# ChristianFeldmann/libHM

Measured on AMD Instinct MI355X. Metric: decoded Mpixels/s (luma), 2160p Main10 reconstruction + loop filters, higher is better.
Workload: dtype int16 samples / int32 accumulate; 1 GPU; 3840x2160 Main10 lowdelay_P pictures, pre-parsed CTU metadata: prep+MC+dequant/IT/recon+deblock+SAO, batch of 16 independent pictures per step, inputs resident in HBM; sub_benchmark=full, streams=2, parallelism=frame-parallel, 1 process per GPU, no data-path collective

## Files before the change

include/hmgpu.h:

```cpp
#ifndef HMGPU_H
#define HMGPU_H

#include <stddef.h>
#include <stdint.h>

#ifdef __cplusplus
extern "C" {
#endif

#define HMGPU_VERSION 1

typedef enum hmgpu_status {
  HMGPU_OK = 0,
  HMGPU_EINVAL = 1,
  HMGPU_EDEVICE = 2,
  HMGPU_EUNSUPPORTED = 3,
  HMGPU_ENOMEM = 4
} hmgpu_status;

#define HMGPU_MAX_REF 16
#define HMGPU_MAX_SLICES 600
#define HMGPU_NO_PIC (-1)

enum { HMGPU_B_SLICE = 0, HMGPU_P_SLICE = 1, HMGPU_I_SLICE = 2 };
// ... 101 lines not shown
void* hmgpu_host_alloc(size_t bytes);
void  hmgpu_host_free(void* p);

int32_t hmgpu_num_ctus(const hmgpu_seq_params* seq);
int32_t hmgpu_parts_per_ctu(const hmgpu_seq_params* seq);

hmgpu_status hmgpu_picture_acquire(hmgpu_ctx* ctx, hmgpu_pic* out);
hmgpu_status hmgpu_picture_release(hmgpu_ctx* ctx, hmgpu_pic pic);
hmgpu_status hmgpu_picture_upload(hmgpu_ctx* ctx, hmgpu_pic pic, const int16_t* const planes[3], const int32_t strides[3]);
hmgpu_status hmgpu_picture_download(hmgpu_ctx* ctx, hmgpu_pic pic, int16_t* const planes[3], const int32_t strides[3]);

hmgpu_status hmgpu_picture_download_begin(hmgpu_ctx* ctx, hmgpu_pic pic, int16_t* const planes[3], const int32_t strides[3], uint64_t* ticket);
hmgpu_status hmgpu_download_wait(hmgpu_ctx* ctx, uint64_t ticket);

hmgpu_status hmgpu_picture_download_packed(hmgpu_ctx* ctx, hmgpu_pic pic, void* const planes[3], const int32_t stride_bytes[3],
                                           int32_t bytes_per_sample, int32_t crop_left, int32_t crop_right, int32_t crop_top, int32_t crop_bottom);
hmgpu_status hmgpu_picture_hash(hmgpu_ctx* ctx, hmgpu_pic pic, int32_t method, uint8_t digest[3][16], int32_t* digest_len);
hmgpu_status hmgpu_picture_hash_begin(hmgpu_ctx* ctx, hmgpu_pic pic, int32_t method , uint64_t* ticket);
hmgpu_status hmgpu_hash_wait(hmgpu_ctx* ctx, uint64_t ticket, int32_t block, uint8_t digest[3][16], int32_t* digest_len, int32_t* ready);

typedef enum { HMGPU_REGION_FINISHED = 0, HMGPU_REGION_RECEIVE = 1 } hmgpu_region;
hmgpu_status hmgpu_picture_transfer(hmgpu_ctx* src, hmgpu_pic src_pic, hmgpu_ctx* dst, hmgpu_pic dst_pic);
uint64_t     hmgpu_transfer_bytes(const hmgpu_ctx* ctx);
hmgpu_status hmgpu_picture_device_region(hmgpu_ctx* ctx, hmgpu_pic pic, int32_t which, void** base, int64_t* bytes);
hmgpu_status hmgpu_picture_commit_received(hmgpu_ctx* ctx, hmgpu_pic pic);
void* hmgpu_stream(hmgpu_ctx* ctx);

enum { HMGPU_EXPORT_PLANAR = 0, HMGPU_EXPORT_SEMIPLANAR = 1, HMGPU_EXPORT_RGB = 2 };
typedef struct hmgpu_export_desc {
  int32_t layout;
  int32_t bit_depth[2];
  int32_t bytes_per_sample;
  int32_t msb_aligned;
  int32_t crop[4];
  int32_t matrix, full_range;
  int32_t reserved[6];
} hmgpu_export_desc;
typedef struct hmgpu_export_plan {
  int32_t planes;
  int32_t width[3], height[3];
  int32_t row_bytes[3];
  int32_t coef[16];
} hmgpu_export_plan;
hmgpu_status hmgpu_export_plan_for(const hmgpu_seq_params* seq, const hmgpu_export_desc* desc, hmgpu_export_plan* out);
hmgpu_status hmgpu_picture_export(hmgpu_ctx* ctx, hmgpu_pic pic, const hmgpu_export_desc* desc, void* const dst[3],
                                  const int64_t pitch_bytes[3], int32_t on_stream, void* stream);
// ... 194 lines not shown
```

libhm_amd/__init__.py:

```python
import ctypes as C
import os

import numpy as np

from . import abi

_HERE = os.path.dirname(os.path.abspath(__file__))
LIB_PATH = os.path.join(_HERE, "libhmgpu.so")
_lib = None


class HmgpuError(RuntimeError):
    def __init__(self, status, what, device_error=0):
        self.status = status
        self.device_error = device_error
        names = {1: "HMGPU_EINVAL", 2: "HMGPU_EDEVICE", 3: "HMGPU_EUNSUPPORTED", 4: "HMGPU_ENOMEM"}
        super().__init__("%s failed: %s%s" % (what, names.get(status, status),
                                              " (hipError %d)" % device_error if status == 2 else ""))


def _share_torch_hip_runtime():
    import importlib.util
    import sys
    if "torch" in sys.modules:
# ... 21 lines not shown
        L = C.CDLL(LIB_PATH)
        L.hmgpu_create.argtypes = [C.POINTER(abi.SeqParams), C.c_int, C.POINTER(C.c_void_p)]
        L.hmgpu_destroy.argtypes = [C.c_void_p]
        L.hmgpu_destroy.restype = None
        L.hmgpu_last_device_error.argtypes = [C.c_void_p]
        L.hmgpu_debug_stall_intra.argtypes = [C.c_void_p, C.c_int32, C.c_int32]
        L.hmgpu_sync.argtypes = [C.c_void_p]
        L.hmgpu_status_string.restype = C.c_char_p
        L.hmgpu_kernel_name.restype = C.c_char_p
        L.hmgpu_num_ctus.argtypes = [C.POINTER(abi.SeqParams)]
        L.hmgpu_parts_per_ctu.argtypes = [C.POINTER(abi.SeqParams)]
        L.hmgpu_picture_acquire.argtypes = [C.c_void_p, C.POINTER(C.c_int32)]
        L.hmgpu_picture_release.argtypes = [C.c_void_p, C.c_int32]
        L.hmgpu_picture_upload.argtypes = [C.c_void_p, C.c_int32, C.POINTER(C.c_void_p), C.POINTER(C.c_int32)]
        L.hmgpu_picture_download.argtypes = [C.c_void_p, C.c_int32, C.POINTER(C.c_void_p), C.POINTER(C.c_int32)]
        L.hmgpu_set_streams.argtypes = [C.c_void_p, C.c_int32]
        L.hmgpu_picture_download_packed.argtypes = [C.c_void_p, C.c_int32, C.POINTER(C.c_void_p), C.POINTER(C.c_int32)] + [C.c_int32] * 5
        L.hmgpu_picture_hash.argtypes = [C.c_void_p, C.c_int32, C.c_int32, C.c_void_p, C.POINTER(C.c_int32)]
        L.hmgpu_picture_device_region.argtypes = [C.c_void_p, C.c_int32, C.c_int32, C.POINTER(C.c_void_p), C.POINTER(C.c_int64)]
        L.hmgpu_picture_commit_received.argtypes = [C.c_void_p, C.c_int32]
        L.hmgpu_picture_transfer.argtypes = [C.c_void_p, C.c_int32, C.c_void_p, C.c_int32]
        L.hmgpu_transfer_bytes.argtypes = [C.c_void_p]
        L.hmgpu_transfer_bytes.restype = C.c_uint64
        L.hmgpu_export_plan_for.argtypes = [C.POINTER(abi.SeqParams), C.POINTER(abi.ExportDesc), C.POINTER(abi.ExportPlan)]
        L.hmgpu_picture_export.argtypes = [C.c_void_p, C.c_int32, C.POINTER(abi.ExportDesc), C.POINTER(C.c_void_p), C.POINTER(C.c_int64),
                                           C.c_int32, C.c_void_p]
        L.hmgpu_export_scaled_plan_for.argtypes = [C.POINTER(abi.SeqParams), C.POINTER(abi.ExportDesc), C.POINTER(abi.ExportScale),
                                                   C.POINTER(abi.ExportPlan)]
        L.hmgpu_export_scale_taps.argtypes = [C.POINTER(abi.SeqParams), C.POINTER(abi.ExportDesc), C.POINTER(abi.ExportScale), C.c_int32,
                                              C.c_int32, C.c_int32, C.POINTER(C.c_int32), C.POINTER(C.c_int32), C.POINTER(C.c_int16)]
        L.hmgpu_picture_export_scaled.argtypes = [C.c_void_p, C.c_int32, C.POINTER(abi.ExportDesc), C.POINTER(abi.ExportScale),
                                                  C.POINTER(C.c_void_p), C.POINTER(C.c_int64), C.c_int32, C.c_void_p]
        L.hmgpu_export_tensor_plan_for.argtypes = [C.POINTER(abi.SeqParams), C.POINTER(abi.ExportDesc), C.POINTER(abi.ExportScale),
                                                   C.POINTER(abi.ExportTensor), C.POINTER(abi.ExportPlan)]
        L.hmgpu_pictures_export.argtypes = [C.c_void_p, C.c_int32, C.POINTER(C.c_int32), C.POINTER(abi.ExportDesc), C.POINTER(abi.ExportScale),
                                            C.POINTER(abi.ExportTensor), C.POINTER(C.c_void_p), C.POINTER(C.c_int64), C.POINTER(C.c_int64),
                                            C.c_int32, C.c_void_p]
        L.hmgpu_export_destination_check.argtypes = [C.c_void_p, C.c_int32, C.POINTER(abi.ExportDesc), C.POINTER(abi.ExportScale),
                                                     C.POINTER(abi.ExportTensor), C.POINTER(C.c_void_p), C.POINTER(C.c_int64),
                                                     C.POINTER(C.c_int64)]
        L.hmgpu_export_windows_plan_for.argtypes = [C.POINTER(abi.SeqParams), C.POINTER(abi.ExportDesc), C.POINTER(abi.ExportScale),
                                                    C.POINTER(abi.ExportTensor), C.c_int32, C.POINTER(abi.ExportWindow),
                                                    C.POINTER(abi.ExportPlan)]
        L.hmgpu_pictures_export_windows.argtypes = [C.c_void_p, C.c_int32, C.POINTER(C.c_int32), C.POINTER(abi.ExportDesc),
                                                    C.POINTER(abi.ExportScale), C.POINTER(abi.ExportTensor), C.POINTER(abi.ExportWindow),
                                                    C.POINTER(C.c_void_p), C.POINTER(C.c_int64), C.POINTER(C.c_int64), C.c_int32, C.c_void_p]
# ... 412 lines not shown

    def picture_hash(self, pic, method):
        dig = (C.c_uint8 * 48)()
        n = C.c_int32()
        self._chk(lib().hmgpu_picture_hash(self._h, pic, method, dig, C.byref(n)), "hmgpu_picture_hash")
        return np.array([dig[16 * k + i] for k in range(3) for i in range(n.value)], dtype=np.uint8)

    def device_region(self, pic, receive=False):
        base, nbytes = C.c_void_p(), C.c_int64()
        self._chk(lib().hmgpu_picture_device_region(self._h, pic, 1 if receive else 0, C.byref(base), C.byref(nbytes)),
                  "hmgpu_picture_device_region")
        return int(base.value), int(nbytes.value)

    def commit_received(self, pic):
        self._chk(lib().hmgpu_picture_commit_received(self._h, pic), "hmgpu_picture_commit_received")

    def transfer_to(self, pic, other, other_pic):
        self._chk(lib().hmgpu_picture_transfer(self._h, pic, other._h, other_pic), "hmgpu_picture_transfer")

    @property
    def transfer_bytes(self):
        return int(lib().hmgpu_transfer_bytes(self._h))

    def stream_handle(self):
        return int(lib().hmgpu_stream(self._h) or 0)

    def decompress_slice(self, pic, slice_idx, slice_params, meta, coeffs, first_ctu=0, num_ctus=None):
        n = self.num_ctus - first_ctu if num_ctus is None else num_ctus
        st = lib().hmgpu_decompress_slice(self._h, pic, slice_idx, C.byref(slice_params), C.byref(meta.struct),
                                          C.byref(coeffs.struct), first_ctu, n)
        self._chk(st, "hmgpu_decompress_slice")

    def filter_picture(self, pic, pic_params, sao_raw=None, stages=7):
        arr = abi.sao_array_from_raw(sao_raw) if sao_raw is not None else None
        st = lib().hmgpu_filter_picture_stages(self._h, pic, C.byref(pic_params), arr, stages)
        self._chk(st, "hmgpu_filter_picture_stages")

    @staticmethod
    def picture_jobs(jobs):
        arr = (abi.PictureJob * len(jobs))()
        arr._keep = [jobs]
        for i, (pic, slices, meta, coeffs) in enumerate(jobs):
            sl = (C.POINTER(abi.SliceParams) * len(slices))(*[C.pointer(s) for s in slices])
            arr._keep.append(sl)
            arr[i].pic, arr[i].num_slices, arr[i].slices = pic, len(slices), sl
            arr[i].meta = C.pointer(meta.struct)
# ... 98 lines not shown
```

libhm_amd/csrc/hmgpu_api.hip:

```cpp
#include "hmgpu_host.h"

#include <algorithm>
#include <cstdio>
#include <cstring>
#include <cstdlib>
#include <new>
#include <vector>

namespace hmgpu_host __attribute__((visibility("hidden"))) {

hipError_t h2d_small(hmgpu_ctx* c, void* dst, const void* src, size_t bytes, hipStream_t hs) {
  const size_t need = (bytes + 63) & ~(size_t)63;
  if (!c->bounce || need > hmgpu_ctx::kBounceSeg) return hipMemcpyAsync(dst, src, bytes, hipMemcpyHostToDevice, hs);
  if (c->bounce_off + need > hmgpu_ctx::kBounceSeg) {
    hipStream_t streams[3] = {c->stream, c->copy_stream, c->copy_stream2};
    for (int k = 0; k < 3; k++) (void)hipEventRecord(c->bounce_ev[c->bounce_seg][k], streams[k]);
    c->bounce_used[c->bounce_seg] = true;
    c->bounce_seg = (c->bounce_seg + 1) % hmgpu_ctx::kBounceSegs;
    c->bounce_off = 0;
    if (c->bounce_used[c->bounce_seg]) for (int k = 0; k < 3; k++) (void)hipEventSynchronize(c->bounce_ev[c->bounce_seg][k]);
  }
  char* at = c->bounce + (size_t)c->bounce_seg * hmgpu_ctx::kBounceSeg + c->bounce_off;
  memcpy(at, src, bytes);
  c->bounce_off += need;
// ... 200 lines not shown
  if (p.derived) hipFree(p.derived);
  p.planes = p.meta = p.coef = p.derived = nullptr; p.pcm = nullptr;
}

hmgpu_status ensure_refs_extended(hmgpu_ctx* c, const Batch& b, size_t call_idx) {
  for (int i = 0; i < b.n; i++) {
    const Picture& p = c->pics[b.pic[i]];
    if (call_idx >= p.calls.size()) continue;
    const SliceDev& sd = p.slices[p.calls[call_idx].slice_idx];
    for (int l = 0; l < 2; l++)
      for (int r = 0; r < HMGPU_MAX_REF; r++)
        if (sd.ref_pic[l][r] >= 0) { hmgpu_status st = ensure_extended(c, sd.ref_pic[l][r]); if (st != HMGPU_OK) return st; }
  }
  return HMGPU_OK;
}

}

namespace hmgpu_host __attribute__((visibility("hidden"))) {

hmgpu_status run_recon(hmgpu_ctx* c, const Batch& b, bool any_intra, bool any_wp, bool any_cells, bool any_bi, bool any_islice) {
  int max_ctus = 0;
  for (int i = 0; i < b.n; i++) max_ctus = std::max(max_ctus, b.num_ctus[i]);
  { ProfScope ps(c, K_PREP); launch_prep(c->d_pics, b, max_ctus, c->parts, any_intra, any_bi, any_cells || c->fmt != 1, c->fmt, c->stream); }
  if (c->fmt != 1) {
    for (int i = 0; i < b.n; i++) {
      const PicDev& d = c->pics[b.pic[i]].dev;
      HIP_TRY(c, hipMemsetAsync(d.resid[1], 0, (size_t)((char*)d.resid[2] - (char*)d.resid[1]) + c->coef_elems[2] * sizeof(int16_t), c->stream));
    }
  }
  McArgs ma;
  memset(&ma, 0, sizeof(ma));
  ma.n = b.n; ma.width = c->seq.width; ma.height = c->seq.height; ma.log2ctu = c->seq.log2_ctu_size; ma.ctus_w = c->ctus_w;
  ma.tw = c->grid_w / 2; ma.npics = c->seq.max_pictures;
  ma.slab = c->plane_slab; ma.pic_stride = 2 * c->plane_bytes; ma.slab_bytes = ma.pic_stride * c->pics.size(); ma.sao_off = (uint32_t)c->plane_bytes;
  for (size_t i = 0; i < c->pics.size(); i++)
    if (c->pics[i].sao_applied) (i < 32 ? ma.sao_mask_lo : ma.sao_mask_hi) |= 1u << (i & 31);
  for (int i = 0; i < b.n; i++) {
    const PicDev& d = c->pics[b.pic[i]].dev;
    ma.first_ctu[i] = b.first_ctu[i]; ma.num_ctus[i] = b.num_ctus[i];
    ma.tmv[i] = d.tmv; ma.slices[i] = d.slices;
  }
  const PicDev& d0 = c->pics[b.pic[0]].dev;
  const char* const base0 = (const char*)c->pics[b.pic[0]].planes;
  uint32_t bps = (uint32_t)std::max(4, std::min(b.n >= 4 ? 12 : 24, max_ctus / 8 + 1));
  {
    ItxArgs ia;
// ... 142 lines not shown
}
const char* hmgpu_kernel_name(int32_t k) { return (k >= 0 && k < HMGPU_NUM_KERNELS) ? kKernelNames[k] : ""; }

int32_t hmgpu_num_ctus(const hmgpu_seq_params* seq) {
  const int c = 1 << seq->log2_ctu_size;
  return ((seq->width + c - 1) / c) * ((seq->height + c - 1) / c);
}
int32_t hmgpu_parts_per_ctu(const hmgpu_seq_params* seq) { return 1 << (2 * seq->log2_ctu_size - 4); }

hmgpu_status hmgpu_create(const hmgpu_seq_params* seq, int device_ordinal, hmgpu_ctx** out) {
  if (!seq || !out) return HMGPU_EINVAL;
  *out = nullptr;
  if (seq->width <= 0 || seq->height <= 0 || (seq->width & 7) || (seq->height & 7)) return HMGPU_EINVAL;
  if (seq->log2_ctu_size < 4 || seq->log2_ctu_size > 6) return HMGPU_EINVAL;
  if (seq->max_pictures < 1 || seq->max_pictures > kMaxPics) return HMGPU_EINVAL;
  if (seq->chroma_format < 0 || seq->chroma_format > 3) return HMGPU_EINVAL;
  if (seq->range_ext_flags & ~(HMGPU_REXT_ROTATION | HMGPU_REXT_IMPLICIT_RDPCM | HMGPU_REXT_EXPLICIT_RDPCM | HMGPU_REXT_INTRA_SMOOTHING_DISABLED)) return HMGPU_EUNSUPPORTED;
  if (seq->bit_depth_luma < 8 || seq->bit_depth_luma > 12 || seq->bit_depth_chroma < 8 || seq->bit_depth_chroma > 12) return HMGPU_EUNSUPPORTED;
  hmgpu_ctx* c = new (std::nothrow) hmgpu_ctx();
  if (!c) return HMGPU_ENOMEM;
  c->seq = *seq;
  c->device = device_ordinal;
  c->host_timing = getenv("HMGPU_HOST_TIMING") != nullptr;
  hipError_t e = hipSetDevice(device_ordinal);
  if (e == hipSuccess) e = hipStreamCreateWithFlags(&c->stream, hipStreamNonBlocking);
  if (e == hipSuccess) e = hipStreamCreateWithFlags(&c->stream2, hipStreamNonBlocking);
  if (e == hipSuccess) e = hipStreamCreateWithFlags(&c->copy_stream, hipStreamNonBlocking);
  if (e == hipSuccess) e = hipStreamCreateWithFlags(&c->copy_stream2, hipStreamNonBlocking);
  if (e == hipSuccess) e = hipEventCreateWithFlags(&c->copy_join, hipEventDisableTiming);
  if (e == hipSuccess) e = hipHostMalloc((void**)&c->bounce, hmgpu_ctx::kBounceSegs * hmgpu_ctx::kBounceSeg, hipHostMallocDefault);
  for (int g = 0; g < hmgpu_ctx::kBounceSegs && e == hipSuccess; g++)
    for (int k = 0; k < 3 && e == hipSuccess; k++) e = hipEventCreateWithFlags(&c->bounce_ev[g][k], hipEventDisableTiming);
  for (int k = 0; k < 8 && e == hipSuccess; k++) e = hipEventCreateWithFlags(&c->copy_ev[k], hipEventDisableTiming);
  for (int k = 0; k < 8 && e == hipSuccess; k++) e = hipEventCreateWithFlags(&c->use_ev[k], hipEventDisableTiming);
  for (int k = 0; k < 32 && e == hipSuccess; k++) e = hipEventCreateWithFlags(&c->dl_ev[k], hipEventDisableTiming | hipEventBlockingSync);
  if (e == hipSuccess) { e = hipHostMalloc((void**)&c->dl_fault, 32 * sizeof(uint32_t), hipHostMallocDefault); if (e == hipSuccess) memset(c->dl_fault, 0, 32 * sizeof(uint32_t)); }
  for (int k = 0; k < 2 && e == hipSuccess; k++) e = hipEventCreateWithFlags(&c->lane_ev[k], hipEventDisableTiming);
  if (e != hipSuccess) { delete c; return HMGPU_EDEVICE; }
  c->ctu = 1 << seq->log2_ctu_size; c->pw = c->ctu / 4; c->parts = c->pw * c->pw;
  c->ctus_w = (seq->width + c->ctu - 1) / c->ctu; c->ctus_h = (seq->height + c->ctu - 1) / c->ctu;
  c->num_ctus = c->ctus_w * c->ctus_h;
  c->grid_w = c->ctus_w * c->pw; c->grid_h = c->ctus_h * c->pw;
  c->fmt = seq->chroma_format == 0 ? 1 : seq->chroma_format;
  c->csx = c->fmt == 3 ? 0 : 1; c->csy = c->fmt == 1 ? 1 : 0;
  c->mx[0] = 128; c->mx[1] = c->mx[2] = 128 >> c->csx;
  c->my[0] = 80; c->my[1] = c->my[2] = 80 >> c->csy;
// ... 264 lines not shown
    int can = 0;
    if (hipDeviceCanAccessPeer(&can, dst->device, src->device) == hipSuccess && can) {
      hipSetDevice(dst->device);
      const hipError_t e = hipDeviceEnablePeerAccess(src->device, 0);
      if (e != hipSuccess && e != hipErrorPeerAccessAlreadyEnabled) return HMGPU_EDEVICE;
      (void)hipGetLastError();
    }
  }
  hipSetDevice(src->device);
  if (!src->xfer_ev[0]) for (int k = 0; k < 2; k++) HIP_TRY(src, hipEventCreateWithFlags(&src->xfer_ev[k], hipEventDisableTiming));
  HIP_TRY(src, hipEventRecord(src->xfer_ev[0], src->stream));
  hipSetDevice(dst->device);
  HIP_TRY(dst, hipStreamWaitEvent(dst->stream, src->xfer_ev[0], 0));
  HIP_TRY(dst, hipMemcpyPeerAsync(to, dst->device, from, src->device, (size_t)n_from, dst->stream));
  HIP_TRY(dst, hipEventRecord(src->xfer_ev[1], dst->stream));
  hipSetDevice(src->device);
  HIP_TRY(src, hipStreamWaitEvent(src->stream, src->xfer_ev[1], 0));
  src->xfer_bytes += (uint64_t)n_from;
  touch(src, src_pic); commit_use(src);
  touch(dst, dst_pic); commit_use(dst);
  return hmgpu_picture_commit_received(dst, dst_pic);
}
uint64_t hmgpu_transfer_bytes(const hmgpu_ctx* c) { return c ? c->xfer_bytes : 0; }

void* hmgpu_stream(hmgpu_ctx* c) { return c ? (void*)c->stream : nullptr; }

hmgpu_status hmgpu_replay_batch(hmgpu_ctx* c, const hmgpu_pic* pics, int32_t n, int32_t stages, int32_t iters) {
  if (!c || !pics || n < 1 || n > kMaxBatch || iters < 0) return HMGPU_EINVAL;
  size_t ncalls = 0;
  for (int i = 0; i < n; i++) {
    if (!valid_pic(c, pics[i])) return HMGPU_EINVAL;
    if (i == 0) ncalls = c->pics[pics[i]].calls.size();
    else if (c->pics[pics[i]].calls.size() != ncalls) return HMGPU_EINVAL;
  }
  if ((stages & 8) && ncalls == 0) return HMGPU_EINVAL;
  hipSetDevice(c->device);
  const int lanes = (c->replay_streams == 2 && n >= 2 && !c->profiling) ? 2 : 1;
  hipStream_t const main_stream = c->stream;
  if (lanes == 2) {
    HIP_TRY(c, hipEventRecord(c->lane_ev[0], main_stream));
    HIP_TRY(c, hipStreamWaitEvent(c->stream2, c->lane_ev[0], 0));
  }
  hmgpu_status result = HMGPU_OK;
  for (int it = 0; it < iters && result == HMGPU_OK; it++) {
    for (int lane = 0; lane < lanes && result == HMGPU_OK; lane++) {
      const int lo = lanes == 2 ? (lane == 0 ? 0 : n / 2) : 0, hi = lanes == 2 ? (lane == 0 ? n / 2 : n) : n;
// ... 144 lines not shown
```

libhm_amd/csrc/hmgpu_dev.h:

```cpp
#pragma once
#include <hip/hip_runtime.h>
#include <stdint.h>
#include "../../include/hmgpu.h"

namespace hmgpu {

constexpr int kMaxBatch = 16;
constexpr int kMaxPics = 64;
constexpr int kTuShards = 8;
constexpr int kCStep = 2;

struct __attribute__((aligned(16))) BlkInfo {
  int16_t mv[2][2];
  int8_t  ref[2];
  int8_t  qp;
  uint8_t flags;
  uint8_t edge;
  uint8_t log2cu;
  uint16_t slice;
};
static_assert(sizeof(BlkInfo) == 16, "BlkInfo must be 16 bytes");

enum : uint8_t {
  BF_VALID = 1,
// ... 173 lines not shown
  if (n <= 8 && (8 % n) == 0) {
    const int m = 8 / n;
    const int per = (nb + m - 1) / m;
    const int x = bid & 7, t = bid >> 3;
    slot = x % n;
    const int r = x / n;
    lb = r * per + t;
    return t < per && lb < nb;
  }
  slot = bid % n; lb = bid / n;
  return lb < nb;
}
__host__ inline int xcd_grid(int n, int nb) {
  if (n <= 8 && (8 % n) == 0) { const int m = 8 / n; return 8 * ((nb + m - 1) / m); }
  return n * nb;
}

struct UnpackArgs {
  int32_t n;
  int32_t pic[kMaxBatch];
  const char* blob[kMaxBatch];
};
void launch_unpack_input(const PicDev* pics, const UnpackArgs& ua, int num_ctus, hipStream_t s);
void launch_prep(const PicDev* pics, const Batch& b, int max_ctus, int parts, bool intra, bool bi, bool write_blk, int fmt, hipStream_t s);
void launch_mc_luma(McArgs& a, int max_ctus, bool wp, bool bi, hipStream_t s);
void launch_mc_chroma(McArgs& a, int max_ctus, bool wp, bool bi, hipStream_t s);
void launch_mc_luma_cells(const PicDev* pics, const PlaneSet* finals, const Batch& b, int max_ctus, int log2ctu, bool wp, hipStream_t s);
void launch_mc_chroma_cells(const PicDev* pics, const PlaneSet* finals, const Batch& b, int max_ctus, int log2ctu, bool wp, hipStream_t s);
void launch_itx(ItxArgs& a, uint32_t blocks_per_shard, hipStream_t s);
void launch_filter_fused(const PicDev* pics, const Batch& b, int width, int height, bool nofilt, hipStream_t s);
void launch_pack(const int16_t* src, int pitch, int step, int x0, int y0, int w, int h, int bytes, uint8_t* dst, int dst_stride, hipStream_t s);
void launch_unpack(const int16_t* src, int w, int h, int16_t* dst, int pitch, int step, hipStream_t s);
void launch_checksum(const int16_t* src, int pitch, int step, int w, int h, int bd, uint32_t* out, hipStream_t s);
struct Md5Batch { int32_t n, pad_; const uint8_t* msg[128]; unsigned long long bytes[128]; uint32_t* out[128]; };
void launch_md5(const Md5Batch& job, hipStream_t s);
void launch_crc(const int16_t* src, int pitch, int step, int w, int h, int bd, uint32_t* rows, uint32_t* out, hipStream_t s);
void launch_intra(const PicDev* pics, const Batch& b, const int32_t* order, int num_ctus, bool lean, hipStream_t s);
constexpr int kMaxExportBatch = 16;
enum { kElemU8 = 0, kElemU16 = 1, kElemF16 = 2, kElemBF16 = 3, kElemF32 = 4 };
template <int ELEM> constexpr int elem_bytes() { return ELEM == kElemU8 ? 1 : ELEM == kElemF32 ? 4 : 2; }
template <int ELEM>
__device__ inline void export_store4(uint8_t* d, const uint32_t v[4], int n, bool vec, int msb, float sc, float bi) {
  uint32_t o[4];
  for (int i = 0; i < 4; i++) {
    if constexpr (ELEM <= kElemU16) {
      o[i] = v[i] << msb;
    } else {
// ... 161 lines not shown
```

libhm_amd/csrc/hmgpu_host.h:

```cpp
#pragma once
#include "hmgpu_dev.h"

#include <atomic>
#include <chrono>
#include <cstring>
#include <unordered_map>
#include <vector>

namespace hmgpu_host __attribute__((visibility("hidden"))) {
using namespace hmgpu;

enum { K_PREP = 0, K_MC_LUMA, K_MC_CHROMA, K_ITX, K_DBK_VER, K_DBK_HOR, K_SAO, K_EXTEND, K_H2D, K_INTRA, K_FILTER, K_UNPACK, K_MC_CELLS };

struct SliceCall { int first_ctu, num_ctus, slice_idx; bool intra, wp, cells, bi, islice, dir; };

struct Picture {
  bool in_use = false;
  bool sao_applied = false;
  bool filter_ready = false;
  bool sao_any = false;
  bool extended = false;
  std::vector<SliceCall> calls;
  void* planes = nullptr;
  void* meta = nullptr;
// ... 74 lines not shown
    int32_t key[8] = {};
    bool valid = false, pending = false;
    uint64_t used = 0;
    char* dev = nullptr;
    char* host = nullptr;
    size_t cap = 0;
    hipEvent_t done = nullptr;
    ScaleClass cls[2];
  };
  static constexpr int kScaleSlots = 8;
  ScaleSlot scale_slot[kScaleSlots];
  uint64_t scale_tick = 0;
  struct WindowBuf {
    char* dev = nullptr;
    char* host = nullptr;
    size_t cap = 0;
    bool pending = false;
    hipEvent_t done = nullptr;
  };
  static constexpr int kWindowBufs = 4;
  WindowBuf window_buf[kWindowBufs];
  int window_next = 0;
  uint64_t xfer_bytes = 0;
  uint32_t* dl_fault = nullptr;
  std::vector<int> touched;
  std::vector<int> intra_launched;
  void* scratch = nullptr;
  size_t scratch_bytes = 0;
  hipEvent_t lane_ev[2] = {nullptr, nullptr};
  int replay_streams = 1;
  int32_t last_err = 0;
  int ctu = 64, pw = 16, parts = 256, ctus_w = 0, ctus_h = 0, num_ctus = 0;
  int fmt = 1, csx = 1, csy = 1;
  int pitch[3] = {0, 0, 0}, rows[3] = {0, 0, 0};
  int mx[3] = {0, 0, 0}, my[3] = {0, 0, 0};
  int grid_w = 0, grid_h = 0;
  uint32_t tu_cap[4] = {0, 0, 0, 0};
  size_t coef_elems[3] = {0, 0, 0};
  std::vector<Picture> pics;
  PicDev* d_pics = nullptr;
  PlaneSet* d_finals = nullptr;
  char* plane_slab = nullptr;
  size_t plane_bytes = 0;
  int32_t* d_ctu_order = nullptr;
  std::vector<PlaneSet> h_finals;
  bool profiling = false;
// ... 62 lines not shown
```

libhm_amd/csrc/k_prep.hip:

```cpp
#include "hmgpu_dev.h"
#include "filter_core.h"

namespace hmgpu {

__constant__ uint8_t c_chroma_scale_420[58] = {
    0, 1, 2, 3, 4, 5, 6, 7, 8, 9, 10, 11, 12, 13, 14, 15, 16, 17, 18, 19, 20, 21, 22, 23, 24, 25, 26, 27, 28, 29,
    29, 30, 31, 32, 33, 33, 34, 34, 35, 35, 36, 36, 37, 37, 38, 39, 40, 41, 42, 43, 44, 45, 46, 47, 48, 49, 50, 51};

__constant__ uint8_t c_chroma422_mode[36] = {
    0, 1, 2, 2, 2, 2, 3, 5, 7, 8, 10, 12, 13, 15, 17, 18, 19, 20, 21, 22, 23, 23, 24, 24, 25, 25, 26, 27, 27, 28, 28, 29, 29, 30, 31, 36};

__device__ inline void qp_param(int qp_y, int comp, int bd, int chroma_off, int fmt, int8_t& per, int8_t& rem) {
  const int bdo = 6 * (bd - 8);
  int base;
  if (comp == 0) base = qp_y + bdo;
  else {
    base = clip3(-bdo, 57, qp_y + chroma_off);
    base = base < 0 ? base + bdo : (fmt == 1 ? c_chroma_scale_420[base] : min(base, 51)) + bdo;
  }
  per = (int8_t)(base / 6);
  rem = (int8_t)(base % 6);
}

struct Quad {
// ... 474 lines not shown
          if (comp && mode == 36) mode = ldg(P.intra_dir[0] + cb + (FMT == 3 ? q.z0 + j : (q.z0 & ~((1 << (2 * (q.log2cu - 2))) - 1))));
          if (FMT == 2 && comp) mode = c_chroma422_mode[mode];
          flags |= (mode == 10 ? 1 : mode == 26 ? 2 : 0) << 3;
        }
      }
    }
    if (FMT == 1 && P.coef_start[0] != nullptr) off = coff[comp] + (comp == 0 ? 16u * __popc(lmask & ((1u << j) - 1u)) : 0u);
    const TuRec r = make_tu(q.gx0 + dx, q.gy0 + dy, comp, flags, xflags, per[comp], rem[comp], off);
    const int c = cls[k];
    const uint32_t i = lds_base[c] + loc[k];
    if (i < P.tu_cap[c]) {
      uint32_t* dst = reinterpret_cast<uint32_t*>(P.tu[c] + (size_t)shard * P.tu_cap[c] + i);
      const uint32_t* src = reinterpret_cast<const uint32_t*>(&r);
      stg(dst, src[0]); stg(dst + 1, src[1]); stg(dst + 2, src[2]);
    }
  }
  __syncthreads();
  if (lds_last) {
    if (threadIdx.x < 4 * kTuShards) stg(P.tu_count + threadIdx.x, atomicExch(&P.tu_work[threadIdx.x], 0u));
    else if (threadIdx.x == 4 * kTuShards) atomicExch(&P.tu_work[4 * kTuShards], 0u);
  }
}

__global__ void k_zero_intra_done(const PicDev* __restrict__ pics, Batch b) {
  const PicDev& P = pics[b.pic[blockIdx.x]];
  for (int i = threadIdx.x; i < 3 * P.num_ctus; i += blockDim.x) stg(P.intra_done + i, 0u);
}

void launch_prep(const PicDev* pics, const Batch& b, int max_ctus, int parts, bool intra, bool bi, bool write_blk, int fmt, hipStream_t s) {
  if (intra) hipLaunchKernelGGL(k_zero_intra_done, dim3((unsigned)b.n), dim3(256), 0, s, pics, b);
  dim3 grid((unsigned)(((size_t)max_ctus * (parts / 4) + 255) / 256), 1, (unsigned)b.n);
  const int wb = write_blk ? 1 : 0;
  if (fmt == 3) hipLaunchKernelGGL((k_prep<3, true, false>), grid, dim3(256), 0, s, pics, b, wb);
  else if (fmt == 2) hipLaunchKernelGGL((k_prep<2, true, false>), grid, dim3(256), 0, s, pics, b, wb);
  else if (parts == 256) {
    if (bi) hipLaunchKernelGGL((k_prep<1, true, true>), grid, dim3(256), 0, s, pics, b, wb);
    else hipLaunchKernelGGL((k_prep<1, false, true>), grid, dim3(256), 0, s, pics, b, wb);
  } else {
    if (bi) hipLaunchKernelGGL((k_prep<1, true, false>), grid, dim3(256), 0, s, pics, b, wb);
    else hipLaunchKernelGGL((k_prep<1, false, false>), grid, dim3(256), 0, s, pics, b, wb);
  }
}

}
```

Measured before the change: 194,600 Mpixels/s.

## Add specialized lean prep kernel for uni-pred 4:2:0 64x64-CTU batches

```diff
diff --git a/include/hmgpu.h b/include/hmgpu.h
--- a/include/hmgpu.h
+++ b/include/hmgpu.h
@@ -147,6 +147,7 @@
 typedef enum { HMGPU_REGION_FINISHED = 0, HMGPU_REGION_RECEIVE = 1 } hmgpu_region;
 hmgpu_status hmgpu_picture_transfer(hmgpu_ctx* src, hmgpu_pic src_pic, hmgpu_ctx* dst, hmgpu_pic dst_pic);
 uint64_t     hmgpu_transfer_bytes(const hmgpu_ctx* ctx);
+uint64_t     hmgpu_prep_lean_launches(const hmgpu_ctx* ctx);
 hmgpu_status hmgpu_picture_device_region(hmgpu_ctx* ctx, hmgpu_pic pic, int32_t which, void** base, int64_t* bytes);
 hmgpu_status hmgpu_picture_commit_received(hmgpu_ctx* ctx, hmgpu_pic pic);
 void* hmgpu_stream(hmgpu_ctx* ctx);
diff --git a/libhm_amd/__init__.py b/libhm_amd/__init__.py
--- a/libhm_amd/__init__.py
+++ b/libhm_amd/__init__.py
@@ -67,6 +67,8 @@
         L.hmgpu_picture_transfer.argtypes = [C.c_void_p, C.c_int32, C.c_void_p, C.c_int32]
         L.hmgpu_transfer_bytes.argtypes = [C.c_void_p]
         L.hmgpu_transfer_bytes.restype = C.c_uint64
+        L.hmgpu_prep_lean_launches.argtypes = [C.c_void_p]
+        L.hmgpu_prep_lean_launches.restype = C.c_uint64
         L.hmgpu_export_plan_for.argtypes = [C.POINTER(abi.SeqParams), C.POINTER(abi.ExportDesc), C.POINTER(abi.ExportPlan)]
         L.hmgpu_picture_export.argtypes = [C.c_void_p, C.c_int32, C.POINTER(abi.ExportDesc), C.POINTER(C.c_void_p), C.POINTER(C.c_int64),
                                            C.c_int32, C.c_void_p]
@@ -525,6 +527,10 @@
     def transfer_bytes(self):
         return int(lib().hmgpu_transfer_bytes(self._h))
 
+    @property
+    def prep_lean_launches(self):
+        return int(lib().hmgpu_prep_lean_launches(self._h))
+
     def stream_handle(self):
         return int(lib().hmgpu_stream(self._h) or 0)
 
diff --git a/libhm_amd/csrc/hmgpu_api.hip b/libhm_amd/csrc/hmgpu_api.hip
--- a/libhm_amd/csrc/hmgpu_api.hip
+++ b/libhm_amd/csrc/hmgpu_api.hip
@@ -246,7 +246,15 @@
 hmgpu_status run_recon(hmgpu_ctx* c, const Batch& b, bool any_intra, bool any_wp, bool any_cells, bool any_bi, bool any_islice) {
   int max_ctus = 0;
   for (int i = 0; i < b.n; i++) max_ctus = std::max(max_ctus, b.num_ctus[i]);
-  { ProfScope ps(c, K_PREP); launch_prep(c->d_pics, b, max_ctus, c->parts, any_intra, any_bi, any_cells || c->fmt != 1, c->fmt, c->stream); }
+  const bool write_blk = any_cells || c->fmt != 1;
+  bool lean = !c->prep_general && c->fmt == 1 && c->parts == 256 && !any_cells && !any_bi && !write_blk;
+  for (int i = 0; i < b.n && lean; i++) {
+    const Picture& p = c->pics[b.pic[i]];
+    if (p.dev.any_nofilt) lean = false;
+    for (const SliceCall& sc : p.calls) if (sc.bi || sc.cells) lean = false;
+  }
+  if (lean) c->prep_lean_launches++;
+  { ProfScope ps(c, K_PREP); launch_prep(c->d_pics, b, max_ctus, c->parts, any_intra, any_bi, write_blk, lean, c->fmt, c->stream); }
   if (c->fmt != 1) {
     for (int i = 0; i < b.n; i++) {
       const PicDev& d = c->pics[b.pic[i]].dev;
@@ -435,6 +443,7 @@
   c->seq = *seq;
   c->device = device_ordinal;
   c->host_timing = getenv("HMGPU_HOST_TIMING") != nullptr;
+  { const char* e = getenv("HMGPU_PREP"); c->prep_general = e && !strcmp(e, "general"); }
   hipError_t e = hipSetDevice(device_ordinal);
   if (e == hipSuccess) e = hipStreamCreateWithFlags(&c->stream, hipStreamNonBlocking);
   if (e == hipSuccess) e = hipStreamCreateWithFlags(&c->stream2, hipStreamNonBlocking);
@@ -745,6 +754,7 @@
   return hmgpu_picture_commit_received(dst, dst_pic);
 }
 uint64_t hmgpu_transfer_bytes(const hmgpu_ctx* c) { return c ? c->xfer_bytes : 0; }
+uint64_t hmgpu_prep_lean_launches(const hmgpu_ctx* c) { return c ? c->prep_lean_launches : 0; }
 
 void* hmgpu_stream(hmgpu_ctx* c) { return c ? (void*)c->stream : nullptr; }
 
diff --git a/libhm_amd/csrc/hmgpu_dev.h b/libhm_amd/csrc/hmgpu_dev.h
--- a/libhm_amd/csrc/hmgpu_dev.h
+++ b/libhm_amd/csrc/hmgpu_dev.h
@@ -219,7 +219,7 @@
   const char* blob[kMaxBatch];
 };
 void launch_unpack_input(const PicDev* pics, const UnpackArgs& ua, int num_ctus, hipStream_t s);
-void launch_prep(const PicDev* pics, const Batch& b, int max_ctus, int parts, bool intra, bool bi, bool write_blk, int fmt, hipStream_t s);
+void launch_prep(const PicDev* pics, const Batch& b, int max_ctus, int parts, bool intra, bool bi, bool write_blk, bool lean, int fmt, hipStream_t s);
 void launch_mc_luma(McArgs& a, int max_ctus, bool wp, bool bi, hipStream_t s);
 void launch_mc_chroma(McArgs& a, int max_ctus, bool wp, bool bi, hipStream_t s);
 void launch_mc_luma_cells(const PicDev* pics, const PlaneSet* finals, const Batch& b, int max_ctus, int log2ctu, bool wp, hipStream_t s);
diff --git a/libhm_amd/csrc/hmgpu_host.h b/libhm_amd/csrc/hmgpu_host.h
--- a/libhm_amd/csrc/hmgpu_host.h
+++ b/libhm_amd/csrc/hmgpu_host.h
@@ -120,6 +120,8 @@
   WindowBuf window_buf[kWindowBufs];
   int window_next = 0;
   uint64_t xfer_bytes = 0;
+  bool prep_general = false;
+  uint64_t prep_lean_launches = 0;
   uint32_t* dl_fault = nullptr;
   std::vector<int> touched;
   std::vector<int> intra_launched;
diff --git a/libhm_amd/csrc/k_prep.hip b/libhm_amd/csrc/k_prep.hip
--- a/libhm_amd/csrc/k_prep.hip
+++ b/libhm_amd/csrc/k_prep.hip
@@ -520,16 +520,365 @@
   }
 }
 
+__device__ inline u32x4 load_ref_row(const SliceDev* s) {
+  const uint32_t* w = reinterpret_cast<const uint32_t*>(&s->ref_pic[0][0]);
+  u32x4 r; r.x = ldu<true>(w); r.y = ldu<true>(w + 1); r.z = ldu<true>(w + 2); r.w = ldu<true>(w + 3);
+  return r;
+}
+__device__ inline uint32_t ref_row_pic(u32x4 row, int r) {
+  const uint32_t lo = (r & 4) ? row.y : row.x, hi = (r & 4) ? row.w : row.z;
+  return (((r & 8) ? hi : lo) >> (8 * (r & 3))) & 0xffu;
+}
+
+__device__ inline u32x2 lean_cell(bool valid, bool intra, uint32_t mvw, int r0, u32x4 refs, uint32_t qp_byte, uint32_t cbf4, int tr) {
+  const uint32_t bits = (((cbf4 >> (tr & 7)) & 0x01010101u) * 0x01020408u) >> 24;
+  const bool use0 = valid && !intra && r0 >= 0;
+  const uint32_t ref = use0 ? ref_row_pic(refs, r0) : 0xffu;
+  u32x2 c;
+  c.x = use0 ? mvw : 0u;
+  c.y = valid ? ref | ((qp_byte & 0xffu) << 8) | ((1u | (intra ? 2u : 0u) | (bits << 2)) << 16) : 0xffu;
+  return c;
+}
+
+__device__ inline u32x2 lean_cell_from_arrays(const PicDev& P, int n, int an, u32x4 refs) {
+  const size_t i = (size_t)n * 256 + (size_t)an * 4;
+  const uint32_t part4 = ldg(reinterpret_cast<const uint32_t*>(P.part_size + i)), tr4 = ldg(reinterpret_cast<const uint32_t*>(P.tr_idx + i));
+  const uint32_t pred4 = ldg(reinterpret_cast<const uint32_t*>(P.pred_mode + i)), cbf4 = ldg(reinterpret_cast<const uint32_t*>(P.cbf[0] + i));
+  const uint32_t qp4 = ldg(reinterpret_cast<const uint32_t*>(P.qp + i)), r04 = ldg(reinterpret_cast<const uint32_t*>(P.ref_idx[0] + i));
+  uint32_t w0 = ldg(reinterpret_cast<const uint32_t*>(P.mv[0]) + i);
+  asm volatile("" : "+v"(w0));
+  return lean_cell((int)(int8_t)(part4 & 0xff) != HMGPU_SIZE_NONE, (int)(int8_t)(pred4 & 0xff) == HMGPU_MODE_INTRA, w0, (int)(int8_t)(r04 & 0xff), refs,
+                   qp4, cbf4, (int)(tr4 & 0xff));
+}
+
+__device__ inline int lean_bs_area(u32x2 p, u32x2 q) {
+  if ((p.y | q.y) & (2u << 16)) return 2;
+  if ((p.y ^ q.y) & 0xffu) return 1;
+  return mvd4(p.x, q.x) ? 1 : 0;
+}
+
+__device__ inline void div6(int base, int8_t& per, int8_t& rem) {
+  const int s = base >> 31, m = (base ^ s) - s, qm = (m * 10923) >> 16, qd = (qm ^ s) - s;
+  per = (int8_t)qd;
+  rem = (int8_t)(base - 6 * qd);
+}
+__device__ inline void qp_param_420(int qp_y, int comp, int bd, int chroma_off, int8_t& per, int8_t& rem) {
+  const int bdo = 6 * (bd - 8);
+  int base;
+  if (comp == 0) base = qp_y + bdo;
+  else {
+    base = clip3(-bdo, 57, qp_y + chroma_off);
+    base = base < 0 ? base + bdo : (int)c_chroma_scale_420[base] + bdo;
+  }
+  div6(base, per, rem);
+}
+
+__global__ void __launch_bounds__(256) k_prep_lean(const PicDev* __restrict__ pics, Batch b) {
+  constexpr int kAbove = 256, kLeft = 256 + 32;
+  __shared__ uint32_t lds_cnt[4], lds_base[4], lds_stat[2], lds_last;
+  __shared__ __attribute__((aligned(8))) u32x2 lds_cell[256 + 32 + 8];
+  const PicDev& P = pics[b.pic[blockIdx.z]];
+  if (threadIdx.x < 4) lds_cnt[threadIdx.x] = 0;
+  if (threadIdx.x < 2) lds_stat[threadIdx.x] = 0;
+  __syncthreads();
+  const int wave_ctu = __builtin_amdgcn_readfirstlane((int)threadIdx.x >> 6);
+  const int ctu_l = (int)blockIdx.x * 4 + wave_ctu;
+  const bool active = ctu_l < b.num_ctus[blockIdx.z];
+  const int a = (int)threadIdx.x & 63;
+  bool valid = false, intra = false;
+  int ctu = 0, z0 = 0, gx0 = 0, gy0 = 0, x4 = 0, y4 = 0, log2cu = 3, log2tu = 3, tr = 0, qp_cu = 0, cb_off = 0, cr_off = 0, ctus_w = 1;
+  uint32_t ts[3] = {0, 0, 0}, bypass = 0, hasm = 0, cnt[3] = {0, 0, 0}, lmask = 0, loc[6] = {}, edge_ver = 0, edge_hor = 0;
+  auto set_has = [&](int k, bool v) { hasm |= (v ? 1u : 0u) << k; };
+  auto has = [&](int k) { return ((hasm >> k) & 1u) != 0; };
+  int cls[6] = {};
+  u32x2 cell; cell.x = 0u; cell.y = 0xffu;
+  if (active) {
+    ctu = b.first_ctu[blockIdx.z] + ctu_l;
+    z0 = a * 4;
+    ctus_w = P.ctus_w;
+    const size_t idx = (size_t)ctu * 256 + z0;
+    const int cx = ctu % ctus_w, cy = ctu / ctus_w;
+    x4 = zscan_x(z0); y4 = zscan_y(z0);
+    gx0 = cx * 16 + x4; gy0 = cy * 16 + y4;
+    const int n_left = cx > 0 ? ctu - 1 : ctu, n_above = cy > 0 ? ctu - ctus_w : ctu;
+    int sidx = 0, sidx_left = 0, sidx_above = 0;
+    if (P.slice_idx) {
+      sidx = (int)ldu<true>(P.slice_idx + ctu);
+      sidx_left = (int)ldu<true>(P.slice_idx + n_left); sidx_above = (int)ldu<true>(P.slice_idx + n_above);
+    }
+    const SliceDev* sl = P.slices + sidx;
+    const u32x4 refs = load_ref_row(sl);
+    const bool deblock_sl = !ldu<true>(&sl->deblocking_disable);
+    const int lf_across_slices = ldu<true>(&sl->lf_across_slices);
+    cb_off = ldu<true>(&sl->cb_qp_offset); cr_off = ldu<true>(&sl->cr_qp_offset);
+    auto ctu_avail = [&](int n, int ns) {
+      bool avail = true;
+      if (!lf_across_slices && P.slice_idx && ns != sidx) avail = false;
+      if (!P.lf_across_tiles && P.tile_idx && ldu<true>(P.tile_idx + n) != ldu<true>(P.tile_idx + ctu)) avail = false;
+      return avail;
+    };
+    const bool avail_left = ctu_avail(n_left, sidx_left), avail_above = ctu_avail(n_above, sidx_above);
+    const uint32_t part4 = ldg(reinterpret_cast<const uint32_t*>(P.part_size + idx));
+    const uint32_t depth4 = ldg(reinterpret_cast<const uint32_t*>(P.depth + idx));
+    const uint32_t pred4 = ldg(reinterpret_cast<const uint32_t*>(P.pred_mode + idx));
+    const uint32_t qp4 = ldg(reinterpret_cast<const uint32_t*>(P.qp + idx));
+    const uint32_t tr4 = ldg(reinterpret_cast<const uint32_t*>(P.tr_idx + idx));
+    const uint32_t byp4 = ldg(reinterpret_cast<const uint32_t*>(P.bypass + idx)), pcm4 = ldg(reinterpret_cast<const uint32_t*>(P.ipcm + idx));
+    const uint32_t r04 = ldg(reinterpret_cast<const uint32_t*>(P.ref_idx[0] + idx));
+    const u32x4 mv0 = ldg4(P.mv[0] + idx * 2);
+    uint32_t cbf[3];
+#pragma unroll
+    for (int c = 0; c < 3; c++) {
+      cbf[c] = ldg(reinterpret_cast<const uint32_t*>(P.cbf[c] + idx));
+      ts[c] = P.tskip[c] ? ldg(reinterpret_cast<const uint32_t*>(P.tskip[c] + idx)) : 0u;
+    }
+    bypass = byp4;
+    {
+      const int t0 = wave_ctu * 64;
+      const bool need_above = cy > 0 && t0 - ctus_w * 64 < 0, need_left = cx > 0 && t0 - 64 < 0;
+      const int sp = (a & 1) | ((a & 2) << 1) | ((a & 4) << 2);
+      auto fetch = [&](int n, int an, int ns) {
+        return lean_cell_from_arrays(P, n, an, load_ref_row(P.slices + ns));
+      };
+      if (need_above && a < 8) lds_cell[kAbove + wave_ctu * 8 + a] = fetch(n_above, sp | 0x2a, sidx_above);
+      if (need_left && a < 8) lds_cell[kLeft + a] = fetch(n_left, (sp << 1) | 0x15, sidx_left);
+    }
+    const int part_size = (int)(int8_t)(part4 & 0xff);
+    valid = gx0 * 4 < P.width && gy0 * 4 < P.height && part_size != HMGPU_SIZE_NONE;
+    tr = tr4 & 0xff;
+    log2cu = 6 - (int)(depth4 & 0xff);
+    log2tu = log2cu - tr;
+    intra = (int)(int8_t)(pred4 & 0xff) == HMGPU_MODE_INTRA;
+    qp_cu = (int)(int8_t)(qp4 & 0xff);
+    const int cu_parts = 1 << (log2cu - 2);
+    const int tu_parts = log2tu > 2 ? 1 << (log2tu - 2) : 1;
+    if (valid && deblock_sl) {
+      const int rx = x4 & (cu_parts - 1), ry = y4 & (cu_parts - 1);
+      {
+        bool filt, trans;
+        if (rx == 0) {
+          bool avail = gx0 != 0;
+          if (avail && x4 == 0) avail = avail_left;
+          filt = trans = avail;
+        } else {
+          trans = x4 == (x4 & ~(tu_parts - 1));
+          bool pu = false;
+          switch (part_size) {
+            case HMGPU_SIZE_Nx2N: case HMGPU_SIZE_NxN: pu = rx == (cu_parts >> 1); break;
+            case HMGPU_SIZE_nLx2N: pu = rx == (cu_parts >> 2); break;
+            case HMGPU_SIZE_nRx2N: pu = rx == cu_parts - (cu_parts >> 2); break;
+            default: break;
+          }
+          filt = trans || pu;
+        }
+        edge_ver = (filt ? BE_VER_FILTER : 0) | (trans ? BE_VER_TRANSFORM : 0);
+      }
+      {
+        bool filt, trans;
+        if (ry == 0) {
+          bool avail = gy0 != 0;
+          if (avail && y4 == 0) avail = avail_above;
+          filt = trans = avail;
+        } else {
+          trans = y4 == (y4 & ~(tu_parts - 1));
+          bool pu = false;
+          switch (part_size) {
+            case HMGPU_SIZE_2NxN: case HMGPU_SIZE_NxN: pu = ry == (cu_parts >> 1); break;
+            case HMGPU_SIZE_2NxnU: pu = ry == (cu_parts >> 2); break;
+            case HMGPU_SIZE_2NxnD: pu = ry == cu_parts - (cu_parts >> 2); break;
+            default: break;
+          }
+          filt = trans || pu;
+        }
+        edge_hor = (filt ? BE_HOR_FILTER : 0) | (trans ? BE_HOR_TRANSFORM : 0);
+      }
+    }
+    const int r0 = (int)(int8_t)(r04 & 0xff);
+    cell = lean_cell(valid, intra, mv0.x, r0, refs, qp4, cbf[0], tr);
+    const bool one_motion = mv0.y == mv0.x && mv0.z == mv0.x && mv0.w == mv0.x && r04 == (r04 & 0xffu) * 0x01010101u;
+    {
+      TileMv tm;
+      tm.ix0 = tm.iy0 = tm.ix1 = tm.iy1 = 0; tm.frac = 0; tm.ref0 = tm.ref1 = 0; tm.flags = 0; tm.ridx = 0; tm.rmask = 0; tm.slice = 0;
+      if (valid && !intra && r0 >= 0 && one_motion) {
+        const int cs = 1 << log2cu;
+        const int cu_x = (gx0 * 4) & ~(cs - 1), cu_y = (gy0 * 4) & ~(cs - 1);
+        int mvx = (int)(int16_t)(mv0.x & 0xffff), mvy = (int)(int16_t)(mv0.x >> 16);
+        mvx = min((P.width + 8 - cu_x - 1) << 2, max((-64 - 8 - cu_x + 1) * 4, mvx));
+        mvy = min((P.height + 8 - cu_y - 1) << 2, max((-64 - 8 - cu_y + 1) * 4, mvy));
+        tm.ix0 = (int16_t)(mvx >> 2); tm.iy0 = (int16_t)(mvy >> 2);
+        tm.frac = (uint8_t)((mvx & 3) | ((mvy & 3) << 2));
+        tm.ref0 = (uint8_t)(cell.y & 0xffu); tm.ridx = (uint8_t)(r0 & 15);
+        tm.flags = TM_ACTIVE;
+        tm.slice = (uint16_t)sidx;
+      }
+      if (valid && !intra && log2tu <= 5) {
+        const uint32_t chain = (1u << (tr + 1)) - 1;
+        uint32_t rm = 0;
+        if (log2tu > 2) rm = ((cbf[0] & 0xff) & chain) == chain ? TR_LUMA : 0;
+        else {
+#pragma unroll
+          for (int j = 0; j < 4; j++) if ((((cbf[0] >> (8 * j)) & 0xff) & chain) == chain) rm |= 1u << j;
+        }
+        if (((cbf[1] & 0xff) & chain) == chain) rm |= TR_CB;
+        if (((cbf[2] & 0xff) & chain) == chain) rm |= TR_CR;
+        tm.rmask = (uint8_t)rm;
+      }
+      stg4(&P.tmv[(size_t)(gy0 >> 1) * (P.grid_w >> 1) + (gx0 >> 1)], __builtin_bit_cast(u32x4, tm));
+    }
+    {
+      const unsigned long long mv_ = __builtin_amdgcn_ballot_w64(valid), mi = __builtin_amdgcn_ballot_w64(valid && intra);
+      const uint32_t ni = (uint32_t)__popcll(mi), nv = (uint32_t)__popcll(mv_);
+      if (a == 0) {
+        stg(P.ctu_intra + ctu, (uint8_t)ni);
+        if (ni) atomicAdd(&lds_stat[0], 4u * ni);
+        if (nv - ni) atomicAdd(&lds_stat[1], 4u * (nv - ni));
+      }
+    }
+    if (valid && log2tu <= 5) {
+      const uint32_t chain = (1u << (tr + 1)) - 1;
+      const bool listed = !intra || (P.has_intra_dir && !(pcm4 & 0xff));
+      if (log2tu > 2) {
+        if ((x4 & (tu_parts - 1)) == 0 && (y4 & (tu_parts - 1)) == 0) {
+          const bool c0 = ((cbf[0] & 0xff) & chain) == chain, c1 = ((cbf[1] & 0xff) & chain) == chain, c2 = ((cbf[2] & 0xff) & chain) == chain;
+          if (c0) cnt[0] = 1u << (2 * log2tu);
+          if (c1) cnt[1] = 1u << (2 * log2tu - 2);
+          if (c2) cnt[2] = 1u << (2 * log2tu - 2);
+          if (listed) {
+            set_has(0, c0); cls[0] = log2tu - 2;
+            set_has(4, c1); cls[4] = log2tu - 3;
+            set_has(5, c2); cls[5] = log2tu - 3;
+          }
+        }
+      } else {
+#pragma unroll
+        for (int j = 0; j < 4; j++) if ((((cbf[0] >> (8 * j)) & 0xff) & chain) == chain) lmask |= 1u << j;
+        const bool c1 = ((cbf[1] & 0xff) & chain) == chain, c2 = ((cbf[2] & 0xff) & chain) == chain;
+        cnt[0] = 16u * __popc(lmask);
+        if (c1) cnt[1] = 16;
+        if (c2) cnt[2] = 16;
+        if (listed) hasm = lmask | (c1 ? 16u : 0u) | (c2 ? 32u : 0u);
+      }
+    }
+  }
+#pragma unroll
+  for (int k = 0; k < 6; k++) if (has(k)) loc[k] = atomicAdd(&lds_cnt[cls[k]], 1u);
+  uint32_t coff[3] = {0, 0, 0};
+  if (P.coef_start[0] != nullptr) {
+#pragma unroll
+    for (int c = 0; c < 3; c++) {
+      uint32_t incl = cnt[c];
+#pragma unroll
+      for (int d = 1; d < 64; d <<= 1) { const uint32_t o = __shfl_up(incl, d); if (a >= d) incl += o; }
+      coff[c] = incl - cnt[c];
+      if (active) coff[c] += ldu<true>(P.coef_start[c] + ctu);
+    }
+  }
+  if (active) lds_cell[threadIdx.x] = cell;
+  __syncthreads();
+  if (active) {
+    EdgeRec er; er.v[0] = er.v[1] = er.h[0] = er.h[1] = 0;
+    const int t0 = wave_ctu * 64;
+    const int q_qp = (int)(int8_t)((cell.y >> 8) & 0xffu);
+    const uint32_t q_bits = (cell.y >> 18) & 15u;
+    if (edge_ver & BE_VER_FILTER) {
+      const int al = (((a & 0x15) - 1) & 0x15) | (a & 0x2a);
+      int at = t0 + al;
+      if (x4 == 0) { at -= 64; if (at < 0) at = kLeft + (y4 >> 1); }
+      const u32x2 p = lds_cell[at];
+      const int bsa = lean_bs_area(p, cell);
+      const uint32_t p_bits = (p.y >> 18) & 15u;
+      const uint32_t pk = (uint32_t)((((int)(int8_t)((p.y >> 8) & 0xffu) + q_qp + 1) >> 1) + 32) << 2;
+      const bool trans = (edge_ver & BE_VER_TRANSFORM) != 0;
+#pragma unroll
+      for (int k = 0; k < 2; k++) {
+        const bool coded = (((p_bits >> (2 * k + 1)) | (q_bits >> (2 * k))) & 1u) != 0;
+        const int bs = bsa == 2 ? 2 : (trans && coded) ? 1 : bsa;
+        er.v[k] = bs ? (uint16_t)((uint32_t)bs | pk) : (uint16_t)0;
+      }
+    }
+    if (edge_hor & BE_HOR_FILTER) {
+      const int au = (((a & 0x2a) - 1) & 0x2a) | (a & 0x15);
+      int at = t0 + au;
+      if (y4 == 0) { at -= ctus_w * 64; if (at < 0) at = kAbove + wave_ctu * 8 + (x4 >> 1); }
+      const u32x2 p = lds_cell[at];
+      const int bsa = lean_bs_area(p, cell);
+      const uint32_t p_bits = (p.y >> 18) & 15u;
+      const uint32_t pk = (uint32_t)((((int)(int8_t)((p.y >> 8) & 0xffu) + q_qp + 1) >> 1) + 32) << 2;
+      const bool trans = (edge_hor & BE_HOR_TRANSFORM) != 0;
+#pragma unroll
+      for (int k = 0; k < 2; k++) {
+        const bool coded = (((p_bits >> (2 + k)) | (q_bits >> k)) & 1u) != 0;
+        const int bs = bsa == 2 ? 2 : (trans && coded) ? 1 : bsa;
+        er.h[k] = bs ? (uint16_t)((uint32_t)bs | pk) : (uint16_t)0;
+      }
+    }
+    stg2(reinterpret_cast<uint32_t*>(P.edges + (size_t)(gy0 >> 1) * (P.grid_w >> 1) + (gx0 >> 1)), __builtin_bit_cast(u32x2, er));
+  }
+  const int shard = blockIdx.x & (kTuShards - 1);
+  if (threadIdx.x < 4) {
+    const uint32_t n = lds_cnt[threadIdx.x];
+    lds_base[threadIdx.x] = n ? atomicAdd(&P.tu_work[threadIdx.x * kTuShards + shard], n) : 0u;
+  } else if (threadIdx.x < 6) {
+    const uint32_t n = lds_stat[threadIdx.x - 4];
+    if (n) atomicAdd(&P.stats[(threadIdx.x - 4) * kTuShards + shard], (unsigned long long)n);
+  }
+  __syncthreads();
+  if (threadIdx.x == 0) lds_last = atomicAdd(&P.tu_work[4 * kTuShards], 1u) == gridDim.x - 1 ? 1u : 0u;
+  constexpr int ctu_luma = 64 * 64;
+  int8_t per[3] = {0, 0, 0}, rem[3] = {0, 0, 0};
+  if (hasm & 15u) qp_param_420(qp_cu, 0, P.bd[0], 0, per[0], rem[0]);
+  if (hasm & 16u) qp_param_420(qp_cu, 1, P.bd[1], cb_off, per[1], rem[1]);
+  if (hasm & 32u) qp_param_420(qp_cu, 2, P.bd[2], cr_off, per[2], rem[2]);
+#pragma unroll
+  for (int k = 0; k < 6; k++) {
+    if (!has(k)) continue;
+    const int comp = k < 4 ? 0 : k - 3;
+    const int j = k < 4 ? k : 0, dx = j & 1, dy = j >> 1, bsize = comp == 0 ? log2tu : max(log2tu - 1, 2);
+    const int tsk = (ts[comp] >> (8 * j)) & 0xff;
+    uint32_t off = comp == 0 ? (uint32_t)ctu * ctu_luma + 16u * (z0 + j) : (uint32_t)ctu * (ctu_luma >> 2) + 4u * z0;
+    int flags = ((comp == 0 && log2tu == 2 && intra) ? 1 : 0) | ((tsk & 1) ? 2 : 0) | ((bypass & 0xff) ? 4 : 0) | (intra ? 32 : 0);
+    int xflags = 0;
+    if ((flags & 6) && P.range_ext) {
+      if (!intra) {
+        if (P.range_ext & HMGPU_REXT_EXPLICIT_RDPCM) flags |= ((tsk >> 1) & 3) << 3;
+      } else {
+        if ((P.range_ext & HMGPU_REXT_ROTATION) && bsize == 2) xflags |= 1;
+        if (P.range_ext & HMGPU_REXT_IMPLICIT_RDPCM) {
+          const size_t cb = (size_t)ctu * 256;
+          int mode = ldg(P.intra_dir[comp ? 1 : 0] + cb + z0 + j);
+          if (comp && mode == 36) mode = ldg(P.intra_dir[0] + cb + (z0 & ~((1 << (2 * (log2cu - 2))) - 1)));
+          flags |= (mode == 10 ? 1 : mode == 26 ? 2 : 0) << 3;
+        }
+      }
+    }
+    if (P.coef_start[0] != nullptr) off = coff[comp] + (comp == 0 ? 16u * __popc(lmask & ((1u << j) - 1u)) : 0u);
+    const TuRec r = make_tu(gx0 + dx, gy0 + dy, comp, flags, xflags, per[comp], rem[comp], off);
+    const int c = cls[k];
+    const uint32_t i = lds_base[c] + loc[k];
+    if (i < P.tu_cap[c]) {
+      uint32_t* dst = reinterpret_cast<uint32_t*>(P.tu[c] + (size_t)shard * P.tu_cap[c] + i);
+      const uint32_t* src = reinterpret_cast<const uint32_t*>(&r);
+      stg(dst, src[0]); stg(dst + 1, src[1]); stg(dst + 2, src[2]);
+    }
+  }
+  __syncthreads();
+  if (lds_last) {
+    if (threadIdx.x < 4 * kTuShards) stg(P.tu_count + threadIdx.x, atomicExch(&P.tu_work[threadIdx.x], 0u));
+    else if (threadIdx.x == 4 * kTuShards) atomicExch(&P.tu_work[4 * kTuShards], 0u);
+  }
+}
+
 __global__ void k_zero_intra_done(const PicDev* __restrict__ pics, Batch b) {
   const PicDev& P = pics[b.pic[blockIdx.x]];
   for (int i = threadIdx.x; i < 3 * P.num_ctus; i += blockDim.x) stg(P.intra_done + i, 0u);
 }
 
-void launch_prep(const PicDev* pics, const Batch& b, int max_ctus, int parts, bool intra, bool bi, bool write_blk, int fmt, hipStream_t s) {
+void launch_prep(const PicDev* pics, const Batch& b, int max_ctus, int parts, bool intra, bool bi, bool write_blk, bool lean, int fmt, hipStream_t s) {
   if (intra) hipLaunchKernelGGL(k_zero_intra_done, dim3((unsigned)b.n), dim3(256), 0, s, pics, b);
   dim3 grid((unsigned)(((size_t)max_ctus * (parts / 4) + 255) / 256), 1, (unsigned)b.n);
   const int wb = write_blk ? 1 : 0;
-  if (fmt == 3) hipLaunchKernelGGL((k_prep<3, true, false>), grid, dim3(256), 0, s, pics, b, wb);
+  if (lean && fmt == 1 && parts == 256 && !bi && !write_blk) hipLaunchKernelGGL(k_prep_lean, grid, dim3(256), 0, s, pics, b);
+  else if (fmt == 3) hipLaunchKernelGGL((k_prep<3, true, false>), grid, dim3(256), 0, s, pics, b, wb);
   else if (fmt == 2) hipLaunchKernelGGL((k_prep<2, true, false>), grid, dim3(256), 0, s, pics, b, wb);
   else if (parts == 256) {
     if (bi) hipLaunchKernelGGL((k_prep<1, true, true>), grid, dim3(256), 0, s, pics, b, wb);
```

Measured after the change: 194,100 Mpixels/s. Within noise of the previous version (-0.3%).
